# TimoLassmann/tagdust

Measured on AMD Instinct MI355X. Metric: reads/s (150 bp, 8-barcode arch), higher is better.
Workload: dtype f32

## Files before the change

tagdust_amd/csrc/td_jit.h:

```cpp
#pragma once
#include <string>
#include <vector>
#include "../../include/tagdust_hip.h"
#include "td_device.h"

struct TdSpecKnobs {
	int block = 512;
	int min_waves = 4;
	int lsum_oob = 1;
	int rt_min = 16;
	int groupcols = 18;
	int groupcols_fwd = 12;
	int prune = 1;
	int prune_sfx = 1;
	int restart = -1;
	int firstseg = -1;
	int trie_sh = 2;
	int profile = 0;
	int prune_stats = -1;
	std::string extra_opts;
};
TdSpecKnobs td_spec_knobs(void);

#define TD_PRUNE_TABLES 16
#define TD_PRUNE_RESTART_MAX 4

struct TdSpecPlan {
	TdSpecKnobs k;
	int S = 0, H = 0, C = 0;
	std::vector<int> col_off, hmm_off;
	std::vector<int> group, group_f;
	std::vector<int> pure_last, drop_m;
	std::vector<int> bw_off;
	int64_t halves = 0;
	std::vector<int> rt, rt_b;
	std::vector<int> base;
	std::vector<float> hi, lo, nv;
	bool trie_on = false;
	int trie_sh = 1, trie_n_share = 0;
	std::vector<int> trie_ord;
	int first_n = 0;
	int prune_segs = 0;
	int sfx_first = 0;
	float prune_z = 0.0f;
	int restart = 0;
};
TdSpecPlan td_spec_plan(const td_model_desc* m, const TdSpecKnobs& k);

float td_spec_prune_z(const td_model_desc* m, int n_seg, int sfx_first);
void td_spec_prune_tables(const td_model_desc* m, const TdSpecPlan& p, int lcap, int stride, std::vector<float>& tab);
void td_spec_layout(TdSpecLayout& L, const TdSpecPlan& p, int lmax);
int td_spec_compile(const td_model_desc* m, const TdSpecPlan& p, int lsum_oob, int window, std::vector<char>& code, std::string& log,
                    uint64_t* key_out = nullptr, bool key_only = false);
int td_spec_compiles_started(void);
```

tagdust_amd/csrc/td_jit.hip:

```cpp
#include <hip/hip_runtime.h>
#include <hip/hiprtc.h>
#include <math.h>
#include <stdio.h>
#include <string.h>
#include <stdlib.h>

#include <atomic>
#include <map>
#include <mutex>
#include <string>
#include <vector>

#include "../../include/tagdust_hip.h"
#include "td_device.h"
#include <unistd.h>
#include <sys/stat.h>
#include <sys/types.h>
#include "td_embedded_src.h"
#include "td_jit.h"

static std::string flit(float v)
{
	if (isinf(v)) return v < 0 ? "(-__builtin_inff())" : "__builtin_inff()";
	if (v != v) return "__builtin_nanf(\"\")";
// ... 78 lines not shown

int first_labels(const td_model_desc* m, int firstseg)
{
	const int H = m->H, n0 = m->n_hmm[0];
	const int mode = firstseg >= 0 ? firstseg : H > 32;
	if (!mode) return 0;
	if (n0 < 2 || n0 >= H) return 0;
	for (int v = 0; v < n0; v++)
		for (int u = 0; u < v; u++) if (m->A[u * H + v] == 1.0f) return 0;
	for (int w = n0; w < H; w++) {
		int c = 0;
		for (int u = 0; u < n0; u++) c += m->A[u * H + w] == 1.0f;
		if (c != 0 && c != n0) return 0;
	}
	return n0;
}

bool read_like(const td_model_desc* m, int j, int co)
{
	if (m->n_hmm[j] != 1 || m->n_col[j] != 1) return false;
	const float* t = m->trans + (size_t)co * 9;
	for (int k = 0; k < 9; k++) if (k != TD_II && k != TD_ISKIP && t[k] > -INFINITY) return false;
	return m->sM[co] == -INFINITY && m->sI[co] > -INFINITY && t[TD_II] > -INFINITY && t[TD_ISKIP] > -INFINITY;
}
}

TdSpecPlan td_spec_plan(const td_model_desc* m, const TdSpecKnobs& k)
{
	TdSpecPlan p;
	const int S = m->S, H = m->H, C = m->C;
	p.k = k; p.S = S; p.H = H; p.C = C;
	p.col_off.resize(S); p.hmm_off.resize(S);
	for (int j = 0, co = 0, ho = 0; j < S; co += m->n_hmm[j] * m->n_col[j], ho += m->n_hmm[j], j++) { p.col_off[j] = co; p.hmm_off[j] = ho; }
	p.group.resize(S); p.group_f.resize(S); p.pure_last.resize(S); p.drop_m.resize(S); p.bw_off.resize(H);
	for (int j = 0; j < S; j++) {
		p.group[j] = group_size(m->n_hmm[j], m->n_col[j], k.groupcols);
		p.group_f[j] = group_size(m->n_hmm[j], m->n_col[j], k.groupcols_fwd > 0 ? k.groupcols_fwd : k.groupcols);
		p.pure_last[j] = pure_last(m, j, p.col_off[j]);
	}
	int cols = 0;
	for (int j = 0; j < S; j++) {
		p.drop_m[j] = m->n_col[j] >= 2 && p.pure_last[j];
		for (int f = 0; f < m->n_hmm[j]; f++) { p.bw_off[p.hmm_off[j] + f] = cols; cols += 2 * (m->n_col[j] - p.pure_last[j]) - p.drop_m[j]; }
	}
	p.halves = cols;
	p.rt.assign(S, 0); p.rt_b.assign(S, 0); p.base.assign(C, 0);
	p.hi.assign(S, 0.0f); p.lo.assign(S, 0.0f); p.nv.assign(S, 0.0f);
	for (int j = 0; j < S; j++) {
		const int pre = rt_prefix(m, j, p.col_off[j], p.base.data(), &p.hi[j], &p.lo[j], &p.nv[j], k.rt_min);
		if (pre > 0) {
			p.group_f[j] = p.group[j];
			p.rt[j] = pre / p.group[j] * p.group[j];
			p.rt_b[j] = p.rt[j];
		} else {
			p.rt_b[j] = rt_prefix(m, j, p.col_off[j], p.base.data(), &p.hi[j], &p.lo[j], &p.nv[j], 2);
		}
	}
	{
		const int sh = k.trie_sh;
		bool on = p.rt[0] > 0 && sh >= 1 && m->n_col[0] >= sh + 2;
		std::vector<int> ord;
		int n_share = 0;
		if (on) {
			const int G = p.group[0], NC0 = m->n_col[0];
			std::map<std::vector<int>, std::vector<int>> cls;
			for (int f = 0; f < p.rt[0]; f++) {
				std::vector<int> key;
				for (int g = NC0 - sh; g < NC0; g++) key.push_back(p.base[(size_t)(p.col_off[0] + f * NC0 + g)]);
				cls[key].push_back(f);
			}
			std::vector<int> left;
			for (auto& kv : cls) {
				const std::vector<int>& v = kv.second;
				const size_t full = v.size() / (size_t)G * (size_t)G;
				for (size_t i = 0; i < full; i++) ord.push_back(v[i]);
				for (size_t i = full; i < v.size(); i++) left.push_back(v[i]);
// ... 22 lines not shown
	return p;
}

static std::string td_spec_model_section(const td_model_desc* m, const TdSpecPlan& p, int lsum_oob, int window)
{
	std::string s;
	char buf[256];
	const int S = m->S, H = m->H, C = m->C;
	int req = 0;
	for (int j = 0; j < S; j++) if (m->seg_type[j] == 'F') req += m->finger_len[j];
	snprintf(buf, sizeof buf, "#define TDS_BLOCK %d\n#define TDS_MIN_WAVES %d\n", p.k.block, p.k.min_waves);
	s += buf;
	snprintf(buf, sizeof buf, "#define TDS_LSUM_OOB %d\n", lsum_oob != 0);
	s += buf;
	snprintf(buf, sizeof buf, "#define TDS_WINDOW %d\n", window != 0);
	s += buf;
	snprintf(buf, sizeof buf, "#define TDS_PROFILE %d\n", p.k.profile);
	s += buf;
	snprintf(buf, sizeof buf, "#define TD_S %d\n#define TD_H %d\n#define TD_C %d\n#define TD_REQ_FINGER %d\n", S, H, C, req);
	s += buf;
	s += "struct GCol { float t[9]; float sM, sI; float eM[5]; float eI[5]; };\n";
	auto int_array = [&](const char* name, const std::vector<int>& v) {
		s += std::string("static constexpr int ") + name + "[" + std::to_string(v.size()) + "] = {";
		for (size_t i = 0; i < v.size(); i++) { s += std::to_string(v[i]); if (i + 1 < v.size()) s += ","; }
		s += "};\n";
	};
	int_array("kNHmm", std::vector<int>(m->n_hmm, m->n_hmm + S)); int_array("kNCol", std::vector<int>(m->n_col, m->n_col + S));
	int_array("kColOff", p.col_off); int_array("kHmmOff", p.hmm_off);
	int_array("kRtB", p.rt_b);
	s += std::string("static constexpr bool kTrieOn = ") + (p.trie_on ? "true" : "false") + ";\n";
	s += "static constexpr int kTrieSH = " + std::to_string(p.trie_sh) + ";\n";
	s += "static constexpr int kTrieNShare = " + std::to_string(p.trie_n_share) + ";\n";
	int_array("kTrieOrd", p.trie_ord);
	int_array("kGroup", p.group); int_array("kGroupF", p.group_f); int_array("kPureLast", p.pure_last); int_array("kDropM", p.drop_m); int_array("kBwOff", p.bw_off);
	int_array("kRt", p.rt); int_array("kBase", p.base);
	auto float_array = [&](const char* name, const std::vector<float>& v) {
		s += std::string("static constexpr float ") + name + "[" + std::to_string(v.size()) + "] = {";
		for (size_t i = 0; i < v.size(); i++) { s += flit(v[i]); if (i + 1 < v.size()) s += ","; }
		s += "};\n";
	};
	float_array("kHi", p.hi); float_array("kLo", p.lo); float_array("kNv", p.nv);
	s += "static constexpr float kSkip[" + std::to_string(S) + "] = {";
	for (int j = 0; j < S; j++) { s += flit(m->skip[j]); if (j + 1 < S) s += ","; }
	s += "};\n";
	s += "static constexpr float kBg[5] = {";
	for (int i = 0; i < 5; i++) { s += flit(m->bg[i]); if (i < 4) s += ","; }
	s += "};\n";
	const float stay_arg = (float)(1.0 - (1.0 / (double)(float)m->avg_len));
	const float exit_arg = (float)(1.0 / (double)(float)m->avg_len);
	s += "static constexpr float kRStay = " + flit(stay_arg == 0.0f ? -INFINITY : (float)log((double)stay_arg)) + ";\n";
	s += "static constexpr float kRExit = " + flit(exit_arg == 0.0f ? -INFINITY : (float)log((double)exit_arg)) + ";\n";
	s += "static constexpr GCol kCols[" + std::to_string(C) + "] = {\n";
	for (int k = 0; k < C; k++) {
		s += " {{";
		for (int t = 0; t < 9; t++) { s += flit(m->trans[k * 9 + t]); if (t < 8) s += ","; }
		s += "}," + flit(m->sM[k]) + "," + flit(m->sI[k]) + ",{";
		for (int e = 0; e < 5; e++) { s += flit(m->eM[k * 5 + e]); if (e < 4) s += ","; }
		s += "},{";
		for (int e = 0; e < 5; e++) { s += flit(m->eI[k * 5 + e]); if (e < 4) s += ","; }
		s += "}},\n";
	}
	s += "};\n";
	s += "static constexpr unsigned kHinfo[" + std::to_string(H) + "] = {";
	for (int h = 0; h < H; h++) {
		const int seg = m->label[h] & 0xFFFF, f = (m->label[h] >> 16) & 0x7FFF;
		unsigned v = (unsigned)(unsigned char)m->seg_type[seg] | ((unsigned)seg << 8) | ((unsigned)f << 16);
		if (m->seg_type[seg] == 'B' && f == m->n_hmm[seg] - 1) v |= 0x80000000u;
// ... 244 lines not shown
```

tagdust_amd/csrc/td_spec_kernel.inc:

```

#ifndef TDS_BLOCK
#define TDS_BLOCK 512
#endif
#ifndef TDS_MIN_WAVES
#define TDS_MIN_WAVES 4
#endif
#define TDS_REG_H 32
#define TDS_WPB (TDS_BLOCK / TD_WAVE)
#define NEG_INF (-__builtin_inff())
#define DEV __device__ __forceinline__

#define MODE_GET_LABEL 1
#define MODE_ARCH_COMP 5
#define OUT_SUCCESS 0
#define OUT_ARCH_MISMATCH 1
#define OUT_TOO_SHORT 2
#define OUT_BAR_FINGER_NOT_FOUND 3
#define OUT_MATCHES_ARTIFACTS 5
#define OUT_LOW_COMPLEXITY 6
#define N_OUTCOME_SLOTS 8
#define TDS_DIAG(k) (N_OUTCOME_SLOTS + 256 + ((k) - 192))

#ifndef TDS_LSUM_OOB
#define TDS_LSUM_OOB 1
// ... 480 lines not shown
		{
			const int ip = (i - 1 >= 1) ? i - 1 : 1;
			xi_n = codes[ip * TD_WAVE + w.lane];
			Pi_n = PBW(ip);
		}
		close_check(p_hi - i); close_check(p_hi - i);
		if (i <= w.len) stair_dispatch<J, RT, K>(gc, fa, Mlo, Mhi, Ilo, Ihi, Pn, mk_mask(c), c, mk_mask(xi), xi);
		c = xi;
		Pn = Pi;
	}
	close_check(p_hi - p_lo); close_check(p_hi - p_lo);
	if (gc >= 0) w.bad |= 32;
	if (TDS_PRUNE_STATS && w.lane == 0) {
		const int st = closed_at >= 0 ? closed_at : p_hi - p_lo;
		atomicAdd(&w.stats[TDS_DIAG(196)], (unsigned long long)st); atomicAdd(&w.stats[TDS_DIAG(197)], 1ull);
		atomicMax(&w.stats[TDS_DIAG(193)], (unsigned long long)st);
	}
	float* rs = w.rs + (int64_t)(kColOff[J] + fa * NC) * 2 * TD_WAVE + w.lane;
#pragma unroll
	for (int g = 0; g < NC; g++) { rs[(2 * g) * TD_WAVE] = Mlo[g]; rs[(2 * g + 1) * TD_WAVE] = Ilo[g]; }
#undef PBW
}

template <int J, int F>
DEV void bwd_stair_rest(const Wv& w, const uint8_t* __restrict__ codes, const float* __restrict__ P, const int p_hi, const int p_lo)
{
	if constexpr (F < kNHmm[J]) {
		bwd_stair<J, false>(w, codes, P, F, p_hi, p_lo);
		bwd_stair_rest<J, F + 1>(w, codes, P, p_hi, p_lo);
	}
}

#define TDS_BWD_BOUNDS(d, pos) { const int k_ = w.len - (pos); wc_q[d] = w.wc[k_ >= 1 ? k_ - 1 : 0]; if (skip_live) wd_q[d] = w.wd[k_ >= 0 ? k_ : 0]; }
#define TDS_BWD_STEP(SPILL_, WANT_CS_) \
		const int xi = xi_q[d_]; \
		const bool tailb = sfx_nb && i < w.sstopS; \
		const float Pi = tailb ? NEG_INF : Pi_q[d_]; \
		if (tailb) Pn = NEG_INF; \
		SV cs; cs.v = cs_q[d_]; cs.z = RT ? false : first; \
		{ \
			const int ip = (i > PD) ? i - PD : 1; \
			xi_q[d_] = codes[ip * TD_WAVE + w.lane]; \
			Pi_q[d_] = p_init ? ((ip == w.len + 1) ? 0.0f : NEG_INF) : P[ip * TD_WAVE + w.lane]; \
			if (!first && (J > 0 || ip == 1)) cs_q[d_] = Cs[ip * TD_WAVE + w.lane]; \
			if (sfx_nb && ip < w.sstopS) { TDS_BWD_BOUNDS(d_, ip) } \
		} \
		const bool want_cs = (WANT_CS_) && !defer_cs; \
		if (i <= w.len) { \
			const BaseMask kc = mk_mask(c), kx = mk_mask(xi); \
_Pragma("unroll") \
			for (int f = 0; f < NF; f++) { \
				const int col0 = kColOff[J] + (RT ? 0 : FL(f)) * NC; \
				const int colr = kColOff[J] + FL(f) * NC; \
				(void)colr; \
				SV Mc[NC], Ic[NC]; \
				if (sfx_nb && tailb) { \
					const int q = col0 + K; \
					if (!((In[f][K] + kCols[q].t[3]) + EMIT_I(q, kc) >= wc_q[d_])) w.bad |= 8; \
				} \
				if constexpr (SHB == 0) { \
					bwd_row<J, RT>(FL(f), Mn[f], In[f], Pn, kc, c, kx, xi, Mc, Ic); \
				} else { \
					 \
					SV Dp_; \
					if (f == 0) { \
						bwd_cols<J, RT, K, K - SHB>(FL(f), Mn[f], In[f], Pn, kc, c, kx, xi, Mc, Ic, Dp_); \
_Pragma("unroll") \
						for (int g = K - SHB; g <= K; g++) { Msh[g] = Mc[g]; Ish[g] = Ic[g]; } \
						Dsh = Dp_; \
					} else { \
_Pragma("unroll") \
						for (int g = K - SHB; g <= K; g++) { Mc[g] = Msh[g]; Ic[g] = Ish[g]; } \
						Dp_ = Dsh; \
					} \
					bwd_cols<J, RT, K - SHB - 1, 0>(FL(f), Mn[f], In[f], Pn, kc, c, kx, xi, Mc, Ic, Dp_); \
				} \
				if (want_cs) { \
_Pragma("unroll") \
					for (int g = K; g >= 0; --g) { \
						const int q = col0 + g; \
						cs = lsum(cs, addv(addc(Mc[g], kCols[q].sM), EM(g, kx, xi))); \
						cs = lsum(cs, addv(addc(Ic[g], kCols[q].sI), EMIT_I(q, kx))); \
					} \
					if (sfx_nb && tailb && skip_live) { if (!(cs.v >= wd_q[d_])) w.bad |= 16; } \
					cs = lsum(cs, addc(sv(Pi), kSkip[J])); \
				} \
				if (SPILL_) { \
					uint8_t* bw = BW + ((int64_t)kBwOff[kHmmOff[J] + FL(f)] * w.lmax + (int64_t)(i - 1) * ROWH) * (TD_WAVE * 4); \
_Pragma("unroll") \
					for (int p = 0; p < NSF / 2; p++) \
						st4(bw + p * (TD_WAVE * 16), w.lane, Mc[2 * p].v, Ic[2 * p].v, Mc[2 * p + 1].v, Ic[2 * p + 1].v); \
					if (NSF & 1) st2(bw + (NSF / 2) * (TD_WAVE * 16), w.lane, Mc[NSF - 1].v, Ic[NSF - 1].v); \
					if (DM) st1(bw + NSF * (TD_WAVE * 8), w.lane, Ic[NS - 1].v); \
				} \
				if (defer_cs && i == 1) {    \
					float* rs_ = w.rs + (int64_t)(kColOff[J] + FL(f) * NC) * 2 * TD_WAVE + w.lane; \
_Pragma("unroll") \
					for (int g = 0; g < NC; g++) { rs_[(2 * g) * TD_WAVE] = Mc[g].v; rs_[(2 * g + 1) * TD_WAVE] = Ic[g].v; } \
				} \
_Pragma("unroll") \
				for (int g = 0; g < NC; g++) { Mn[f][g] = Mc[g].v; In[f][g] = Ic[g].v; } \
			} \
			if (want_cs) Cs[i * TD_WAVE + w.lane] = cs.v; \
		} \
		c = xi; \
		Pn = Pi;

template <int J, int NF, bool RT, int SHB = 0>
DEV void bwd_group(const Wv& w, const uint8_t* __restrict__ codes, const float* __restrict__ P,
                   float* __restrict__ Cs, uint8_t* __restrict__ BW, const int f0)
{
	constexpr bool defer_cs = kTrieOn && (J == 0);
	constexpr bool permuted = kTrieOn && (J == 0) && RT;
#define FL(f_) (permuted ? kTrieOrd[f0 + (f_)] : f0 + (f_))
	const bool first = (f0 == 0);
	SV Msh[kNCol[J]], Ish[kNCol[J]], Dsh = sv_none();
	(void)Msh; (void)Ish; (void)Dsh;
#define EM(gcol, mask, xval) (RT ? emit_rt(kBase[colr + (gcol)], kHi[J], kLo[J], kNv[J], mask, xval) : EMIT_M(col0 + (gcol), mask))
	constexpr int NC = kNCol[J];
	constexpr int K = NC - 1;
	constexpr int NS = NC - kPureLast[J];
	constexpr int DM = kDropM[J];
	constexpr int NSF = NS - DM;
	constexpr int ROWH = 2 * NS - DM;
	constexpr bool skip_live = LIVE(kSkip[J]);
	float Mn[NF][NC], In[NF][NC];
#pragma unroll
	for (int f = 0; f < NF; f++) {
#pragma unroll
		for (int g = 0; g < NC; g++) { Mn[f][g] = NEG_INF; In[f][g] = NEG_INF; }
	}
	if (TDS_RESTART && J < kPruneSegs && w.rb_on) {
#pragma unroll
		for (int f = 0; f < NF; f++) {
			const float* rs = w.rs + (int64_t)(kColOff[J] + FL(f) * NC) * 2 * TD_WAVE + w.lane;
#pragma unroll
			for (int g = 0; g < NC; g++) { Mn[f][g] = rs[(2 * g) * TD_WAVE]; In[f][g] = rs[(2 * g + 1) * TD_WAVE]; }
		}
	}
	constexpr bool p_init = (J == TD_S - 1);
#define PBW(pos) (p_init ? (((pos) == w.len + 1) ? 0.0f : NEG_INF) : P[(pos) * TD_WAVE + w.lane])
	const bool resumed = TDS_RESTART && (J < kPruneSegs) && w.rb_on;
	const int istart = resumed ? w.cutS + J * (w.rW + 1) : w.tmax;
	int c = resumed ? (int)codes[(istart + 1) * TD_WAVE + w.lane] : 0;
	float Pn = PBW(istart + 1);
	constexpr int PD = pf_dist(NF * NC, RT);
	int xi_q[PD];
	float Pi_q[PD], cs_q[PD];
	float wc_q[PD], wd_q[PD];
	constexpr bool sfx_nb = (kSfxFirst < TD_S) && (J == kSfxFirst - 1);
#pragma unroll
	for (int d = 0; d < PD; d++) {
		const int ip = (istart - d >= 1) ? istart - d : 1;
		xi_q[d] = codes[ip * TD_WAVE + w.lane];
		Pi_q[d] = PBW(ip);
		cs_q[d] = first ? NEG_INF : Cs[ip * TD_WAVE + w.lane];
		wc_q[d] = 0.0f; wd_q[d] = 0.0f;
		if (sfx_nb && ip < w.sstopS) { TDS_BWD_BOUNDS(d, ip) }
	}

	const int ilow = (J >= kSfxFirst) ? w.sstopS : 1;
	if constexpr (PD > 1) {
		int base = istart;
		for (; base - (PD - 1) >= ilow; base -= PD) {
#pragma unroll
			for (int d_ = 0; d_ < PD; d_++) {
				const int i = base - d_;
				{ TDS_BWD_STEP((J >= kPruneSegs || i <= w.cutS || i == 1), ((J > 0) || i == 1)) }
			}
		}
#pragma unroll
		for (int d_ = 0; d_ < PD - 1; d_++) {
			const int i = base - d_;
			if (i >= ilow) { TDS_BWD_STEP((J >= kPruneSegs || i <= w.cutS || i == 1), ((J > 0) || i == 1)) }
		}
	} else {
		constexpr int d_ = 0;
		int i = istart;
		if (J < kPruneSegs) {
			for (; i > w.cutS && i >= 2 && i >= ilow; --i) { TDS_BWD_STEP(false, (J > 0)) }
		}
		for (; i >= ilow; --i) { TDS_BWD_STEP(true, ((J > 0) || i == 1)) }
	}
#undef EM
#undef PBW
#undef FL
}

template <int J, int F, bool RT>
DEV void fold_first_hmm(const Wv& w, const int fa, const int x1, const BaseMask& kx, const float Pi, SV& cs)
{
#define EM(gcol, mask, xval) (RT ? emit_rt(kBase[colr + (gcol)], kHi[J], kLo[J], kNv[J], mask, xval) : EMIT_M(col0 + (gcol), mask))
	constexpr int NC = kNCol[J];
	const int col0 = kColOff[J] + (RT ? 0 : fa) * NC;
	const int colr = kColOff[J] + fa * NC;
	(void)colr;
	const float* rs = w.rs + (int64_t)(kColOff[J] + fa * NC) * 2 * TD_WAVE + w.lane;
	float M[NC], I[NC];
#pragma unroll
	for (int g = 0; g < NC; g++) { M[g] = rs[(2 * g) * TD_WAVE]; I[g] = rs[(2 * g + 1) * TD_WAVE]; }
#pragma unroll
	for (int g = NC - 1; g >= 0; --g) {
		const int q = col0 + g;
		cs = lsum(cs, addv(addc(sv(M[g]), kCols[q].sM), EM(g, kx, x1)));
		cs = lsum(cs, addv(addc(sv(I[g]), kCols[q].sI), EMIT_I(q, kx)));
	}
	cs = lsum(cs, addc(sv(Pi), kSkip[J]));
#undef EM
}
template <int J, int F>
DEV void fold_first_rest(const Wv& w, const int x1, const BaseMask& kx, const float Pi, SV& cs)
{
	if constexpr (F < kNHmm[J]) {
		fold_first_hmm<J, F, false>(w, F, x1, kx, Pi, cs);
		fold_first_rest<J, F + 1>(w, x1, kx, Pi, cs);
// ... 201 lines not shown
		const float Pm = Pm_n;
		{
			const int ip = (i + 1 < q_hi) ? i + 1 : i;
			c_n = codes[ip * TD_WAVE + w.lane];
			Pm_n = P[(ip - 1) * TD_WAVE + w.lane];
		}
		close_check(i - q_lo); close_check(i - q_lo);
		fstair_dispatch<J, 0>(gc, Mlo, Mhi, Ilo, Ihi, Pm, mk_mask(c));
	}
	close_check(q_hi - q_lo); close_check(q_hi - q_lo);
	if (gc < NC) w.bad |= 32;
	if (TDS_PRUNE_STATS && w.lane == 0) {
		const int st = closed_at >= 0 ? closed_at : q_hi - q_lo;
		atomicAdd(&w.stats[TDS_DIAG(194)], (unsigned long long)st); atomicAdd(&w.stats[TDS_DIAG(195)], 1ull);
		atomicMax(&w.stats[TDS_DIAG(192)], (unsigned long long)st);
	}
	float* rs = w.rs + (int64_t)kColOff[J] * 2 * TD_WAVE + w.lane;
#pragma unroll
	for (int g = 0; g < NC; g++) { rs[(2 * g) * TD_WAVE] = Mlo[g]; rs[(2 * g + 1) * TD_WAVE] = Ilo[g]; }
}

template <int J, int NF, bool RT>
DEV void fwd_group(const Wv& w, const uint8_t* __restrict__ codes, const float* __restrict__ P,
                   float* __restrict__ Cs, const float* __restrict__ PB, const uint8_t* __restrict__ BW,
                   float* __restrict__ DP, float* __restrict__ TOTAL, const float b, const int f0)
{
	const bool first = (f0 == 0);
#define EM(gcol, mask, xval) (RT ? emit_rt(kBase[colr + (gcol)], kHi[J], kLo[J], kNv[J], mask, xval) : EMIT_M(col0 + (gcol), mask))
	constexpr int NC = kNCol[J];
	constexpr int K = NC - 1;
	constexpr bool pure = kPureLast[J] != 0;
	constexpr int NS = NC - kPureLast[J];
	constexpr int DM = kDropM[J];
	constexpr int NSF = NS - DM;
	constexpr int ROWH = 2 * NS - DM;
	constexpr int NQ = NSF / 2;
	constexpr int NT = NSF & 1;
	constexpr bool skip_live = LIVE(kSkip[J]);
	float Mp[NF][NC], Ip[NF][NC], tot[NF];
#pragma unroll
	for (int f = 0; f < NF; f++) {
		tot[f] = NEG_INF;
#pragma unroll
		for (int g = 0; g < NC; g++) { Mp[f][g] = NEG_INF; Ip[f][g] = NEG_INF; }
	}
	if (TDS_RESTART && J >= kSfxFirst && w.rf_on) {
		const float* rs = w.rs + (int64_t)kColOff[J] * 2 * TD_WAVE + w.lane;
#pragma unroll
		for (int g = 0; g < NC; g++) { Mp[0][g] = rs[(2 * g) * TD_WAVE]; Ip[0][g] = rs[(2 * g + 1) * TD_WAVE]; }
	}
	constexpr bool p_init = (J == 0);
	const bool resumed = TDS_RESTART && (J >= kSfxFirst) && w.rf_on;
	const int i0 = resumed ? w.sstop - (TD_S - 1 - J) * (w.rWf + 1) : 1;
	float Pm = p_init ? 0.0f : P[(i0 - 1) * TD_WAVE + w.lane];
	constexpr int PD = pf_dist(NF * NC, RT);
	const int pmax = (w.tmax >= 1) ? w.tmax : 1;
	int c_q[PD];
	float Pi_q[PD], cs_q[PD], pb_q[PD], bm_q[PD], ik_q[PD][NF];
	int ba_q[PD];
	float MB_q[PD][NF][NSF + 1], IB_q[PD][NF][NSF + 1];
	constexpr bool pb_init = (J == TD_S - 1);
#define PBR(pos) (pb_init ? (((pos) == w.len + 1) ? 0.0f : NEG_INF) : PB[(pos) * TD_WAVE + w.lane])
#define BWROW(f_, pos_) (BW + ((int64_t)kBwOff[kHmmOff[J] + f0 + (f_)] * w.lmax + (int64_t)((pos_) - 1) * ROWH) * (TD_WAVE * 4))
#define TDS_FWD_FILL(d, p_raw) { \
		const int p_ = ((p_raw) <= pmax) ? (p_raw) : pmax; \
		c_q[d] = codes[p_ * TD_WAVE + w.lane]; \
		Pi_q[d] = p_init ? NEG_INF : P[p_ * TD_WAVE + w.lane]; \
		if (!first) cs_q[d] = Cs[p_ * TD_WAVE + w.lane]; \
		if (pure) pb_q[d] = PBR(p_ + 1); \
		if (own_sum && !first) { bm_q[d] = w.bm[p_ * TD_WAVE + w.lane]; ba_q[d] = w.ba[p_ * TD_WAVE + w.lane]; } \
		const bool rows_ = !((J >= kSfxFirst) && p_ < w.sstop);    \
_Pragma("unroll") \
		for (int f = 0; f < NF; f++) { \
			if (DM && rows_) ik_q[d][f] = ld1(BWROW(f, p_) + NSF * (TD_WAVE * 8), w.lane); \
			if (PD > 1 && rows_) { \
_Pragma("unroll") \
				for (int q = 0; q < NQ; q++) { \
					MB_q[d][f][2 * q] = ldk(BWROW(f, p_) + q * (TD_WAVE * 16), w.lane, 16, 0); IB_q[d][f][2 * q] = ldk(BWROW(f, p_) + q * (TD_WAVE * 16), w.lane, 16, 1); \
					MB_q[d][f][2 * q + 1] = ldk(BWROW(f, p_) + q * (TD_WAVE * 16), w.lane, 16, 2); IB_q[d][f][2 * q + 1] = ldk(BWROW(f, p_) + q * (TD_WAVE * 16), w.lane, 16, 3); \
				} \
				if (NT) { MB_q[d][f][NSF - 1] = ldk(BWROW(f, p_) + NQ * (TD_WAVE * 16), w.lane, 8, 0); IB_q[d][f][NSF - 1] = ldk(BWROW(f, p_) + NQ * (TD_WAVE * 16), w.lane, 8, 1); } \
			} \
		} \
	}
	constexpr bool own_sum = (J == 0) && (kFirstN > 0);
	float lacc[NF];
	uint32_t mbits[NF];
#pragma unroll
	for (int f = 0; f < NF; f++) { lacc[f] = 0.0f; mbits[f] = 0u; }
#pragma unroll
	for (int d = 0; d < PD; d++) {
		cs_q[d] = NEG_INF; pb_q[d] = 0.0f; bm_q[d] = -1.0f; ba_q[d] = 0;
#pragma unroll
		for (int f = 0; f < NF; f++) ik_q[d][f] = NEG_INF;
		TDS_FWD_FILL(d, i0 + d)
	}

	const int iend = (J < kPruneSegs && w.cut < w.tmax) ? w.cut : w.tmax;
	const int itail = (J == kPruneSegs && kPruneSegs > 0) ? w.cut + 1 : w.tmax + 1;
	(void)itail;
	if (i0 > 1 && kMaskDP && !own_sum) {
#pragma unroll
		for (int f = 0; f < NF; f++) {
			if (w.lane == 0) for (int wd = 0; wd < ((i0 - 1) >> 5); wd++) w.pmask[(kHmmOff[J] + f0 + f) * w.nwm + wd] = 0u;
			mbits[f] = 0u;
		}
	}
// ... 71 lines not shown
					lsum2(M, addc(sv(Mp[f][g - 1]), kCols[qp].t[0]), I, addc(sv(Ip[f][g]), kCols[q].t[3]));
					lsum2(M, addc(sv(Ip[f][g - 1]), kCols[qp].t[4]), I, addc(sv(Mp[f][g]), kCols[q].t[1]));
					SV D = addc(Mc[g - 1], kCols[qp].t[2]);
					lsum2(M, addc(Dc, kCols[qp].t[6]), D, addc(Dc, kCols[qp].t[5]));
					M = addv(M, EM(g, kc, c));
					I = addv(I, EMIT_I(q, kc));
					if (want_cs) { cs = lsum(cs, addc(M, kCols[q].t[7])); cs = lsum(cs, addc(I, kCols[q].t[8])); }
					Mc[g] = M; Ic[g] = I; Dc = D;
				}
				if (tail && skip_live) { if (!(cs.v >= uload(w.wb, i))) w.bad |= 2; }
				if (want_cs) cs = lsum(cs, addc(PiS, kSkip[J]));
				if (!sfx_skip) {
				float MB[NC], IB[NC];
#pragma unroll
				for (int p = 0; p < NQ; p++) {
					const f32x4 v = cb[f][p];
					MB[2 * p] = v.x; IB[2 * p] = v.y; MB[2 * p + 1] = v.z; IB[2 * p + 1] = v.w;
				}
				if (NT) { MB[NSF - 1] = ct[f].x; IB[NSF - 1] = ct[f].y; }
				if constexpr (DM != 0) {
					constexpr int g = K - 1;
					const int q = col0 + g;
					const bool nxt = i < w.len;
					const int cx = (i < w.tmax) ? c_n : 0;
					const BaseMask kn = mk_mask(cx);
					SV MnK = addc(sv(pb_n), kCols[col0 + K].t[7]);
					if (!MnK.z) MnK.v = nxt ? MnK.v : NEG_INF;
					const float InK = nxt ? ik_n[f] : NEG_INF;
					SV Mr = addc(addv(MnK, EM(K, kn, cx)), kCols[q].t[0]);
					Mr = lsum(Mr, addc(sv(pb), kCols[q].t[7]));
					Mr = lsum(Mr, addc(addv(sv(InK), EMIT_I(q, kn)), kCols[q].t[1]));
					MB[g] = Mr.v; IB[g] = ik[f];
				}
				if (pure) {
					MB[K] = pb + kCols[col0 + K].t[7];
					IB[K] = pb + kCols[col0 + K].t[8];
				}
				constexpr bool want_tt = kNHmm[J] > 1;
				SV acc = sv_none(), tt = sv(tot[f]);
#pragma unroll
				for (int g = 0; g <= K; ++g) {
					const SV pm = subv(addv(Mc[g], MB[g]), b);
					if (want_tt && g == 0) tt = lsum(tt, pm);
					acc = lsum(acc, pm);
					if (want_tt && g == 0) tt = lsum(tt, subv(addv(addv(addc(PmS, kCols[col0].sI), ei0), IB[0]), b));
					acc = lsum(acc, subv(addv(Ic[g], IB[g]), b));
				}
				if (want_tt) tot[f] = tt.v;
				if (own_sum) {
					lacc[f] = post_prob(acc.v) + lacc[f];
					if (lacc[f] > bm) { bm = lacc[f]; ba = h; }
				} else if (kMaskDP) {
					lpost[f] = acc.v;
				} else {
					DP[((int64_t)(i - 1) * TD_H + h) * TD_WAVE + w.lane] = post_prob(acc.v);
				}
				}
#pragma unroll
				for (int g = 0; g < NC; g++) { Mp[f][g] = Mc[g].v; Ip[f][g] = Ic[g].v; }
			}
			if (want_cs) Cs[i * TD_WAVE + w.lane] = cs.v;
			if (own_sum) { w.bm[i * TD_WAVE + w.lane] = bm; w.ba[i * TD_WAVE + w.lane] = (uint8_t)ba; }
		}
		if (kMaskDP && !own_sum) {
#pragma unroll
			for (int f = 0; f < NF; f++) {
// ... 49 lines not shown
template <int J, int F0>
DEV void fwd_groups(const Wv& w, const uint8_t* __restrict__ codes, const float* __restrict__ P,
                    float* __restrict__ Cs, const float* __restrict__ PB, const uint8_t* __restrict__ BW,
                    float* __restrict__ DP, float* __restrict__ TOTAL, const float b)
{
	if constexpr (TDS_RESTART && F0 == 0 && J >= kSfxFirst) {
		if (w.rf_on) {
			const int q_hi = w.sstop - (TD_S - 1 - J) * (w.rWf + 1);
			fwd_stair<J>(w, codes, P, q_hi - w.rWf, q_hi);
		}
	}
	if constexpr (F0 == 0 && kRt[J] > 0) {
		for (int f0 = 0; f0 < kRt[J]; f0 += kGroupF[J]) fwd_group<J, kGroupF[J], true>(w, codes, P, Cs, PB, BW, DP, TOTAL, b, f0);
		fwd_groups<J, kRt[J]>(w, codes, P, Cs, PB, BW, DP, TOTAL, b);
	} else if constexpr (F0 < kNHmm[J]) {
		constexpr int NF = cmin(kGroupF[J], kNHmm[J] - F0);
		fwd_group<J, NF, false>(w, codes, P, Cs, PB, BW, DP, TOTAL, b, F0);
		fwd_groups<J, F0 + NF>(w, codes, P, Cs, PB, BW, DP, TOTAL, b);
	}
}

template <int J>
DEV void fwd_segments(const Wv& w, const uint8_t* __restrict__ codes, float* __restrict__ SF, const float* __restrict__ SB,
                      int rowlen, const uint8_t* __restrict__ BW, float* __restrict__ DP, float* __restrict__ TOTAL, const float b)
{
	if constexpr (J < TD_S) {
		fwd_groups<J, 0>(w, codes, SF + (int64_t)J * rowlen, SF + (int64_t)(J + 1) * rowlen, SB + (int64_t)(J + 1) * rowlen,
		                 BW, DP, TOTAL, b);
		if (TDS_PROFILE == 2 && J < 8) { const long long t_ = (long long)__builtin_readcyclecounter(); if (w.lane == 0) atomicAdd(&w.stats[TDS_DIAG(216 + J)], (unsigned long long)(t_ - *w.tprof)); *w.tprof = t_; }
		fwd_segments<J + 1>(w, codes, SF, SB, rowlen, BW, DP, TOTAL, b);
	}
}

constexpr bool path_word_trivial(int k)
{
	for (int b = 0; b < 4; b++) {
		const int v = kFirstN + 4 * k + b;
		if (v < TD_H && (kPredFirst[v] != 0 || kPredOff2[v + 1] != kPredOff2[v])) return false;
	}
	return true;
}
constexpr uint32_t path_word_identity(int k)
{
	uint32_t w = 0;
	for (int b = 0; b < 4; b++) w |= (uint32_t)((kFirstN + 4 * k + b) & 0xFF) << (8 * b);
	return w;
}

DEV int prune_scan(const float thr, const int len, const int tmax, const float* __restrict__ fbt, const float* __restrict__ bwt)
{
	int cl = 1;
	for (int i0 = 2; i0 <= tmax; i0 += TDS_SCAN_B) {
		float g[TDS_SCAN_B];
#pragma unroll
		for (int k = 0; k < TDS_SCAN_B; k++) {
			const int i = i0 + k;
			const int mm = (i <= len) ? len - i : 0;
			g[k] = bwt[mm];
		}
		__builtin_amdgcn_sched_barrier(0);
#pragma unroll
		for (int k = 0; k < TDS_SCAN_B; k++) g[k] = uload(fbt, i0 + k) + g[k];
#pragma unroll
		for (int k = 0; k < TDS_SCAN_B; k++) {
			const int i = i0 + k;
			if (i <= len && i <= tmax && g[k] > thr) cl = i;
		}
	}
#pragma unroll
	for (int o = 32; o >= 1; o >>= 1) cl = max(cl, __shfl_xor(cl, o));
	return __builtin_amdgcn_readfirstlane(cl);
}

DEV float leading_bwd_bound(const Wv& w, const int i)
{
	float hb = NEG_INF;
	for (int k0 = 0; i + 1 + k0 <= w.tmax + 1; k0 += TDS_SCAN_B) {
		float q[TDS_SCAN_B];
// ... 369 lines not shown
						if (f != n - 1) n0 = (t > n0) ? t : n0;
						n1 = lsum(n1, t);
					}
					n0 = n0 - n1;
					n2 = n2 + n0;
				}
				hc += n;
			}
			bar_prob = (gg || n2 > 0.0f) ? 0.0f : n2;
		}

		float Q;
		{
			float pbest = lsum(f_score, r_score);
			const double t = ((double)bar_prob + (double)f_score) - (double)pbest;
			const float tf = (float)t;
			const float e = (tf == NEG_INF) ? 0.0f : (float)exp((double)tf);
			pbest = (float)(1.0 - (double)e);
			if (pbest == 0.0f) Q = 40.0f;
			else if (pbest == 1.0f) Q = 0.0f;
			else Q = (float)(-10.0 * log10((double)pbest));
		}
		if (dead || len < 1) Q = 0.0f;

#define BMROW(pos) ((kPruneSegs > 0 && (pos) > w.cut) ? w.cut : (pos))
		int read_type = 0, barcode = -1, fingerprint = -1;
		const int nw1 = ka.nw1;
		uint32_t* keep = ka.out_keep + (int64_t)tile * nw1 * TD_WAVE;

		if (ka.mode == MODE_GET_LABEL) {
			int8_t* labels = ka.out_labels + (int64_t)tile * (ka.out_lmax + 1) * TD_WAVE;
			constexpr int F1 = kFirstN;
			constexpr int HL = H - F1;
			constexpr int PWL = (HL + 3) / 4;
			TDS_PHASE(3);
			if constexpr (HL <= TDS_REG_H) {
				float acc[HL];
	#pragma unroll
				for (int v = 0; v < HL; v++) acc[v] = 0.0f;
				constexpr int LD = TDS_LDP;
				float dq[LD][HL];
				uint32_t mq[LD];
				uint32_t mw[HL];
				auto mask_words = [&](const int word) __attribute__((always_inline)) {
					uint32_t t[HL];
#pragma unroll
					for (int v = 0; v < HL; v++) t[v] = w.pmask[(F1 + v) * w.nwm + word];
					__builtin_amdgcn_sched_barrier(0);
#pragma unroll
					for (int v = 0; v < HL; v++) mw[v] = (uint32_t)__builtin_amdgcn_readfirstlane((int)t[v]);
				};
#pragma unroll
				for (int v = 0; v < HL; v++) mw[v] = 0xFFFFFFFFu;
				if (kMaskDP && tmax >= 1) mask_words(0);
				const int rmax = (tmax >= 1) ? tmax - 1 : 0;
				auto request = [&](auto dtag, auto leadtag, const int p) __attribute__((always_inline)) {
					constexpr int d = decltype(dtag)::v;
					constexpr bool with_lead = decltype(leadtag)::v != 0;
					const int nb = p - 1;
					if (kMaskDP && (nb & 31) == 0 && nb > 0 && nb < tmax) mask_words(nb >> 5);
					const int row = (nb < rmax) ? nb : rmax;
					const float* dpn = DP + ((int64_t)row * H + F1) * TD_WAVE + lane;
					uint32_t bits = 0;
#pragma unroll
					for (int v = 0; v < HL; v++) {
						if (with_lead || !label_leading(F1 + v)) {
							dq[d][v] = dpn[v * TD_WAVE];
// ... 26 lines not shown
					constexpr int d = decltype(dtag)::v;
					float dc[HL];
#pragma unroll
					for (int v = 0; v < HL; v++) dc[v] = dq[d][v];
					const uint32_t mc = mq[d];
					const float bm_c = bm_q[d];
					const int ba_c = ba_q[d];
					if (decltype(reqtag)::v) { request(dtag, leadtag, i + LD); request_bm(dtag, i + LD); }
					uint32_t pws[PWL > 0 ? PWL : 1];
#pragma unroll
					for (int k = 0; k < PWL; k++) pws[k] = 0u;
					if (i <= len) {
						uint32_t pw = 0;
	#pragma unroll
						for (int v = HL - 1; v >= 0; v--) {
							float m = -1.0f;
							int mv = 0;
							if (F1 > 0 && kPredFirst[F1 + v]) {
								const bool gt = bm_p > m;
								m = gt ? bm_p : m;
								mv = gt ? ba_p : mv;
							}
	#pragma unroll
							for (int p = kPredOff2[F1 + v]; p < kPredOff2[F1 + v + 1]; p++) {
								const int u = kPredIdx2[p] - F1;
								const bool gt = acc[u] > m;
								m = gt ? acc[u] : m;
								mv = gt ? u + F1 : mv;
							}
							const bool st = acc[v] >= m;
							m = st ? acc[v] : m;
							mv = st ? v + F1 : mv;
							acc[v] = (((mc >> v) & 1u) ? dc[v] : 0.0f) + m;
							pw |= (uint32_t)mv << (8 * (v & 3));
							if ((v & 3) == 0) { pws[v >> 2] = pw; pw = 0; }
						}
					}
					uint32_t* pathi = PATH + (int64_t)(i - 1) * PWL * TD_WAVE + lane;
#pragma unroll
					for (int k = 0; k < PWL; k++) if (!path_word_trivial(k)) pathi[k * TD_WAVE] = pws[k];
					bm_p = bm_c; ba_p = ba_c;
				};
				{
					auto step_a = [&](auto dtag, const int i) __attribute__((always_inline)) { dp_step(dtag, IC<1>{}, IC<1>{}, i); };
					auto step_b = [&](auto dtag, const int i) __attribute__((always_inline)) { dp_step(dtag, IC<0>{}, IC<1>{}, i); };
					auto step_r = [&](auto dtag, const int i) __attribute__((always_inline)) { dp_step(dtag, IC<0>{}, IC<0>{}, i); };
					int base = 1;
					for (; base + LD - 1 <= tmax && (kPruneSegs == 0 || base + LD <= w.cut); base += LD) ring_block<LD, 0>(step_a, base);
					for (; base + LD - 1 <= tmax; base += LD) ring_block<LD, 0>(step_b, base);
					ring_rest<LD, 0>(step_r, base, tmax);
				}
				TDS_PHASE(4);
				{
					float m = -1.0f;
					int move = 0;
					if (F1 > 0 && len >= 1) {
						const float bl = w.bm[BMROW(len) * TD_WAVE + lane];
						if (bl > m) { m = bl; move = w.ba[BMROW(len) * TD_WAVE + lane]; }
					}
	#pragma unroll
					for (int v = 0; v < HL; v++) {
						const bool gt = acc[v] > m;
						m = gt ? acc[v] : m;
						move = gt ? v + F1 : move;
					}
					if (len >= 1) labels[len * TD_WAVE + lane] = (int8_t)move;
					constexpr int LDT = TDS_LDT;
					uint32_t wq[LDT][PWL > 0 ? PWL : 1];
					auto request_path = [&](auto dtag, const int r) __attribute__((always_inline)) {
						constexpr int d = decltype(dtag)::v;
						const int rc = (r >= 0) ? r : 0;
#pragma unroll
						for (int k = 0; k < PWL; k++)
							wq[d][k] = path_word_trivial(k) ? path_word_identity(k) : PATH[((int64_t)rc * PWL + k) * TD_WAVE + lane];
					};
					auto tb_step = [&](auto dtag, auto reqtag, const int r) __attribute__((always_inline)) {
						constexpr int d = decltype(dtag)::v;
						uint32_t wc[PWL > 0 ? PWL : 1];
#pragma unroll
						for (int k = 0; k < PWL; k++) wc[k] = wq[d][k];
						if (decltype(reqtag)::v) request_path(dtag, r - LDT);
						const int i = r + 1;
						if (i <= len) {
							if (move >= F1) {
								const int ml = move - F1;
								uint32_t pwv = wc[0];
	#pragma unroll
								for (int k = 1; k < PWL; k++) pwv = ((ml >> 2) == k) ? wc[k] : pwv;
								move = (pwv >> (8 * (ml & 3))) & 0xFF;
							}
							labels[(i - 1) * TD_WAVE + lane] = (int8_t)move;
						}
					};
					if (tmax >= 1) {
						auto fillp = [&](auto dtag, const int nr) __attribute__((always_inline)) { request_path(dtag, -nr); };
						auto step_w = [&](auto dtag, const int nr) __attribute__((always_inline)) { tb_step(dtag, IC<1>{}, -nr); };
						auto step_r = [&](auto dtag, const int nr) __attribute__((always_inline)) { tb_step(dtag, IC<0>{}, -nr); };
						int nbase = -(tmax - 1);
						ring_block<LDT, 0>(fillp, nbase);
						for (; nbase + LDT - 1 <= 0; nbase += LDT) ring_block<LDT, 0>(step_w, nbase);
						ring_rest<LDT, 0>(step_r, nbase, 0);
					}
				}

			} else {
				float* const ACCB = (float*)(w.slot + lay.acc);
				uint8_t* PATH8 = (uint8_t*)PATH;
				for (int v = 0; v < HL; v++) ACCB[v * TD_WAVE + lane] = 0.0f;
				float bm_p = 0.0f;
				int ba_p = 0;
				for (int i = 1; i <= tmax; i++) {
					if (i <= len) {
						const float* __restrict__ a0 = ACCB + (int64_t)((i - 1) & 1) * HL * TD_WAVE + lane;
						float* __restrict__ a1 = ACCB + (int64_t)(i & 1) * HL * TD_WAVE + lane;
						const float* __restrict__ dpi = DP + ((int64_t)(i - 1) * H + F1) * TD_WAVE + lane;
						uint8_t* __restrict__ pathi = PATH8 + (int64_t)(i - 1) * HL * TD_WAVE + lane;
						constexpr int CH = 8;
						for (int r = 0; r < kNRuns; r++) {
// ... 327 lines not shown
```

Before: 82.32 million.

## Trim backward row storage, skip length checks in full region, shrink traceback path words

Read-like segments (single column with only insert self-loop and skip) now store only their insert half in the backward row buffer, which shrinks the per-row footprint and the matching loads in the forward/posterior pass. The backward loop is split so that rows below the tile's minimum length run a variant without the per-step length guard. The Viterbi traceback path encoding leaves out a leading run of labels that have no predecessors, so fewer path words are written and read. All of this adds more loop variants and code size, and the index offsets must be exactly right to stay correct.

```diff
diff --git a/tagdust_amd/csrc/td_jit.h b/tagdust_amd/csrc/td_jit.h
--- a/tagdust_amd/csrc/td_jit.h
+++ b/tagdust_amd/csrc/td_jit.h
@@ -31,6 +31,7 @@
 	std::vector<int> col_off, hmm_off;
 	std::vector<int> group, group_f;
 	std::vector<int> pure_last, drop_m;
+	std::vector<int> half_i;
 	std::vector<int> bw_off;
 	int64_t halves = 0;
 	std::vector<int> rt, rt_b;
diff --git a/tagdust_amd/csrc/td_jit.hip b/tagdust_amd/csrc/td_jit.hip
--- a/tagdust_amd/csrc/td_jit.hip
+++ b/tagdust_amd/csrc/td_jit.hip
@@ -134,7 +134,7 @@
 	p.k = k; p.S = S; p.H = H; p.C = C;
 	p.col_off.resize(S); p.hmm_off.resize(S);
 	for (int j = 0, co = 0, ho = 0; j < S; co += m->n_hmm[j] * m->n_col[j], ho += m->n_hmm[j], j++) { p.col_off[j] = co; p.hmm_off[j] = ho; }
-	p.group.resize(S); p.group_f.resize(S); p.pure_last.resize(S); p.drop_m.resize(S); p.bw_off.resize(H);
+	p.group.resize(S); p.group_f.resize(S); p.pure_last.resize(S); p.drop_m.resize(S); p.half_i.resize(S); p.bw_off.resize(H);
 	for (int j = 0; j < S; j++) {
 		p.group[j] = group_size(m->n_hmm[j], m->n_col[j], k.groupcols);
 		p.group_f[j] = group_size(m->n_hmm[j], m->n_col[j], k.groupcols_fwd > 0 ? k.groupcols_fwd : k.groupcols);
@@ -143,7 +143,8 @@
 	int cols = 0;
 	for (int j = 0; j < S; j++) {
 		p.drop_m[j] = m->n_col[j] >= 2 && p.pure_last[j];
-		for (int f = 0; f < m->n_hmm[j]; f++) { p.bw_off[p.hmm_off[j] + f] = cols; cols += 2 * (m->n_col[j] - p.pure_last[j]) - p.drop_m[j]; }
+		p.half_i[j] = !p.pure_last[j] && read_like(m, j, p.col_off[j]);
+		for (int f = 0; f < m->n_hmm[j]; f++) { p.bw_off[p.hmm_off[j] + f] = cols; cols += 2 * (m->n_col[j] - p.pure_last[j]) - p.drop_m[j] - p.half_i[j]; }
 	}
 	p.halves = cols;
 	p.rt.assign(S, 0); p.rt_b.assign(S, 0); p.base.assign(C, 0);
@@ -232,7 +233,7 @@
 	s += "static constexpr int kTrieSH = " + std::to_string(p.trie_sh) + ";\n";
 	s += "static constexpr int kTrieNShare = " + std::to_string(p.trie_n_share) + ";\n";
 	int_array("kTrieOrd", p.trie_ord);
-	int_array("kGroup", p.group); int_array("kGroupF", p.group_f); int_array("kPureLast", p.pure_last); int_array("kDropM", p.drop_m); int_array("kBwOff", p.bw_off);
+	int_array("kGroup", p.group); int_array("kGroupF", p.group_f); int_array("kPureLast", p.pure_last); int_array("kDropM", p.drop_m); int_array("kHalfI", p.half_i); int_array("kBwOff", p.bw_off);
 	int_array("kRt", p.rt); int_array("kBase", p.base);
 	auto float_array = [&](const char* name, const std::vector<float>& v) {
 		s += std::string("static constexpr float ") + name + "[" + std::to_string(v.size()) + "] = {";
diff --git a/tagdust_amd/csrc/td_spec_kernel.inc b/tagdust_amd/csrc/td_spec_kernel.inc
--- a/tagdust_amd/csrc/td_spec_kernel.inc
+++ b/tagdust_amd/csrc/td_spec_kernel.inc
@@ -536,7 +536,7 @@
 }
 
 #define TDS_BWD_BOUNDS(d, pos) { const int k_ = w.len - (pos); wc_q[d] = w.wc[k_ >= 1 ? k_ - 1 : 0]; if (skip_live) wd_q[d] = w.wd[k_ >= 0 ? k_ : 0]; }
-#define TDS_BWD_STEP(SPILL_, WANT_CS_) \
+#define TDS_BWD_STEP(SPILL_, WANT_CS_, FULL_) \
 		const int xi = xi_q[d_]; \
 		const bool tailb = sfx_nb && i < w.sstopS; \
 		const float Pi = tailb ? NEG_INF : Pi_q[d_]; \
@@ -550,7 +550,7 @@
 			if (sfx_nb && ip < w.sstopS) { TDS_BWD_BOUNDS(d_, ip) } \
 		} \
 		const bool want_cs = (WANT_CS_) && !defer_cs; \
-		if (i <= w.len) { \
+		if ((FULL_) || i <= w.len) { \
 			const BaseMask kc = mk_mask(c), kx = mk_mask(xi); \
 _Pragma("unroll") \
 			for (int f = 0; f < NF; f++) { \
@@ -595,7 +595,7 @@
 					for (int p = 0; p < NSF / 2; p++) \
 						st4(bw + p * (TD_WAVE * 16), w.lane, Mc[2 * p].v, Ic[2 * p].v, Mc[2 * p + 1].v, Ic[2 * p + 1].v); \
 					if (NSF & 1) st2(bw + (NSF / 2) * (TD_WAVE * 16), w.lane, Mc[NSF - 1].v, Ic[NSF - 1].v); \
-					if (DM) st1(bw + NSF * (TD_WAVE * 8), w.lane, Ic[NS - 1].v); \
+					if (DM || IH) st1(bw + NSF * (TD_WAVE * 8), w.lane, Ic[NS - 1].v); \
 				} \
 				if (defer_cs && i == 1) {    \
 					float* rs_ = w.rs + (int64_t)(kColOff[J] + FL(f) * NC) * 2 * TD_WAVE + w.lane; \
@@ -625,8 +625,9 @@
 	constexpr int K = NC - 1;
 	constexpr int NS = NC - kPureLast[J];
 	constexpr int DM = kDropM[J];
-	constexpr int NSF = NS - DM;
-	constexpr int ROWH = 2 * NS - DM;
+	constexpr int IH = kHalfI[J];
+	constexpr int NSF = NS - DM - IH;
+	constexpr int ROWH = 2 * NS - DM - IH;
 	constexpr bool skip_live = LIVE(kSkip[J]);
 	float Mn[NF][NC], In[NF][NC];
 #pragma unroll
@@ -664,27 +665,48 @@
 	}
 
 	const int ilow = (J >= kSfxFirst) ? w.sstopS : 1;
+	constexpr int ifull_lo = (J > 0) ? 1 : 2;
 	if constexpr (PD > 1) {
 		int base = istart;
-		for (; base - (PD - 1) >= ilow; base -= PD) {
+		for (; base - (PD - 1) >= ilow && !(base <= w.tmin && (J >= kPruneSegs || base <= w.cutS)); base -= PD) {
 #pragma unroll
 			for (int d_ = 0; d_ < PD; d_++) {
 				const int i = base - d_;
-				{ TDS_BWD_STEP((J >= kPruneSegs || i <= w.cutS || i == 1), ((J > 0) || i == 1)) }
+				{ TDS_BWD_STEP((J >= kPruneSegs || i <= w.cutS || i == 1), ((J > 0) || i == 1), false) }
+			}
+		}
+		for (; base - (PD - 1) >= ilow && base - (PD - 1) >= ifull_lo; base -= PD) {
+#pragma unroll
+			for (int d_ = 0; d_ < PD; d_++) {
+				const int i = base - d_;
+				{ TDS_BWD_STEP(true, (J > 0), true) }
+			}
+		}
+		if constexpr (J == 0) {
+			for (; base - (PD - 1) >= ilow; base -= PD) {
+#pragma unroll
+				for (int d_ = 0; d_ < PD; d_++) {
+					const int i = base - d_;
+					{ TDS_BWD_STEP((J >= kPruneSegs || i <= w.cutS || i == 1), ((J > 0) || i == 1), false) }
+				}
 			}
 		}
 #pragma unroll
 		for (int d_ = 0; d_ < PD - 1; d_++) {
 			const int i = base - d_;
-			if (i >= ilow) { TDS_BWD_STEP((J >= kPruneSegs || i <= w.cutS || i == 1), ((J > 0) || i == 1)) }
+			if (i >= ilow) { TDS_BWD_STEP((J >= kPruneSegs || i <= w.cutS || i == 1), ((J > 0) || i == 1), false) }
 		}
 	} else {
 		constexpr int d_ = 0;
 		int i = istart;
 		if (J < kPruneSegs) {
-			for (; i > w.cutS && i >= 2 && i >= ilow; --i) { TDS_BWD_STEP(false, (J > 0)) }
-		}
-		for (; i >= ilow; --i) { TDS_BWD_STEP(true, ((J > 0) || i == 1)) }
+			for (; i > w.cutS && i >= 2 && i >= ilow; --i) { TDS_BWD_STEP(false, (J > 0), false) }
+		}
+		for (; i > w.tmin && i >= ilow; --i) { TDS_BWD_STEP(true, ((J > 0) || i == 1), false) }
+		for (; i >= ilow && i >= ifull_lo; --i) { TDS_BWD_STEP(true, (J > 0), true) }
+		if constexpr (J == 0) {
+			for (; i >= ilow; --i) { TDS_BWD_STEP(true, ((J > 0) || i == 1), false) }
+		}
 	}
 #undef EM
 #undef PBW
@@ -952,8 +974,9 @@
 	constexpr bool pure = kPureLast[J] != 0;
 	constexpr int NS = NC - kPureLast[J];
 	constexpr int DM = kDropM[J];
-	constexpr int NSF = NS - DM;
-	constexpr int ROWH = 2 * NS - DM;
+	constexpr int IH = kHalfI[J];
+	constexpr int NSF = NS - DM - IH;
+	constexpr int ROWH = 2 * NS - DM - IH;
 	constexpr int NQ = NSF / 2;
 	constexpr int NT = NSF & 1;
 	constexpr bool skip_live = LIVE(kSkip[J]);
@@ -992,7 +1015,7 @@
 		const bool rows_ = !((J >= kSfxFirst) && p_ < w.sstop);    \
 _Pragma("unroll") \
 		for (int f = 0; f < NF; f++) { \
-			if (DM && rows_) ik_q[d][f] = ld1(BWROW(f, p_) + NSF * (TD_WAVE * 8), w.lane); \
+			if ((DM || IH) && rows_) ik_q[d][f] = ld1(BWROW(f, p_) + NSF * (TD_WAVE * 8), w.lane); \
 			if (PD > 1 && rows_) { \
 _Pragma("unroll") \
 				for (int q = 0; q < NQ; q++) { \
@@ -1130,6 +1153,7 @@
 					Mr = lsum(Mr, addc(addv(sv(InK), EMIT_I(q, kn)), kCols[q].t[1]));
 					MB[g] = Mr.v; IB[g] = ik[f];
 				}
+				if constexpr (IH != 0) { MB[0] = NEG_INF; IB[0] = ik[f]; }
 				if (pure) {
 					MB[K] = pb + kCols[col0 + K].t[7];
 					IB[K] = pb + kCols[col0 + K].t[8];
@@ -1245,10 +1269,19 @@
 	}
 }
 
+constexpr bool label_has_pred(int v) { return kPredFirst[v] != 0 || kPredOff2[v + 1] != kPredOff2[v]; }
+constexpr int path_t0()
+{
+	int t = 0;
+	while (kFirstN + t < TD_H && !label_has_pred(kFirstN + t)) t++;
+	for (int v = kFirstN + t; v < TD_H; v++) if (!label_has_pred(v)) return 0;
+	return t;
+}
+constexpr int kPathT0 = path_t0();
 constexpr bool path_word_trivial(int k)
 {
 	for (int b = 0; b < 4; b++) {
-		const int v = kFirstN + 4 * k + b;
+		const int v = kFirstN + kPathT0 + 4 * k + b;
 		if (v < TD_H && (kPredFirst[v] != 0 || kPredOff2[v + 1] != kPredOff2[v])) return false;
 	}
 	return true;
@@ -1256,7 +1289,7 @@
 constexpr uint32_t path_word_identity(int k)
 {
 	uint32_t w = 0;
-	for (int b = 0; b < 4; b++) w |= (uint32_t)((kFirstN + 4 * k + b) & 0xFF) << (8 * b);
+	for (int b = 0; b < 4; b++) w |= (uint32_t)((kFirstN + kPathT0 + 4 * k + b) & 0xFF) << (8 * b);
 	return w;
 }
 
@@ -1692,7 +1725,8 @@
 			int8_t* labels = ka.out_labels + (int64_t)tile * (ka.out_lmax + 1) * TD_WAVE;
 			constexpr int F1 = kFirstN;
 			constexpr int HL = H - F1;
-			constexpr int PWL = (HL + 3) / 4;
+			constexpr int T0 = (HL <= TDS_REG_H) ? kPathT0 : 0;
+			constexpr int PWL = (HL - T0 + 3) / 4;
 			TDS_PHASE(3);
 			if constexpr (HL <= TDS_REG_H) {
 				float acc[HL];
@@ -1785,8 +1819,10 @@
 							m = st ? acc[v] : m;
 							mv = st ? v + F1 : mv;
 							acc[v] = (((mc >> v) & 1u) ? dc[v] : 0.0f) + m;
-							pw |= (uint32_t)mv << (8 * (v & 3));
-							if ((v & 3) == 0) { pws[v >> 2] = pw; pw = 0; }
+							if (v >= T0) {
+								pw |= (uint32_t)mv << (8 * ((v - T0) & 3));
+								if (((v - T0) & 3) == 0) { pws[(v - T0) >> 2] = pw; pw = 0; }
+							}
 						}
 					}
 					uint32_t* pathi = PATH + (int64_t)(i - 1) * PWL * TD_WAVE + lane;
@@ -1835,8 +1871,8 @@
 						if (decltype(reqtag)::v) request_path(dtag, r - LDT);
 						const int i = r + 1;
 						if (i <= len) {
-							if (move >= F1) {
-								const int ml = move - F1;
+							if (move >= F1 + T0) {
+								const int ml = move - F1 - T0;
 								uint32_t pwv = wc[0];
 	#pragma unroll
 								for (int k = 1; k < PWL; k++) pwv = ((ml >> 2) == k) ? wc[k] : pwv;
```

New measurement: 82.11 million. About the same (-0.3%).
